# chorowski-lab/pytorch-asr

Hardware: AMD Instinct MI355X
Metric: CTC train-step frames/sec (higher is better)
Workload: dtype bf16; 1 GPU; WSJ mono-char CTC (egs/wsj/yamls/ctc.yaml shapes), DeepSpeech2 conv+4xBiLSTM-320 encoder + FSTDecoder, fwd+bwd+GradientClipping(clip 480000, skip 4.8e+06 = recipe x global_batch/16)+PolyakDecay+Adam, synthetic 40-dim x 1-channel x 1000-frame fbank; batch_per_gpu=768, global_batch=768, frames=1000, classes=49, parallelism=dp1, batch_norm=per-replica statistics, optimizer_steps=139, step_boundary=device: att_speech.fused_step (clip / skip decision + Adam, no read-back)

## Files before the change

### include/asr_amd.h

```cpp
#ifndef ASR_AMD_H
#define ASR_AMD_H

#include <stdint.h>

#ifdef __cplusplus
extern "C" {
#endif

enum {
    ASR_OK = 0,
    ASR_EINVAL = 1,
    ASR_EUNSUPPORTED = 2,
    ASR_ELAUNCH = 3
};

int asr_abi_version(void);

const char *asr_strerror(int code);

int64_t asr_lattice_fwbw_workspace_bytes(int T, int B, int C, int N);

int asr_lattice_fwbw_f32(const float *lp, int T, int B, int C,
                         const int32_t *lens,
                         const int32_t *src_in, const int32_t *il_in,
// ... 56 lines not shown
int asr_lattice_grouped_fwbw_f32(
    const float *lp, int T, int B, int C, const int32_t *lens, int N, int G, int Wg, int Wh,
    const int32_t *g_of, const int32_t *h_of, const int32_t *label, const int32_t *selfx,
    const int32_t *uniq, const int32_t *mem_g, const int32_t *mem_h, const float *term,
    float neg_inf, float *out_logZ, float *out_grad, float *out_logZ_bwd, void *workspace,
    int64_t workspace_bytes, void *stream);
int asr_lattice_grouped_fwbw_acc_f32(
    const float *lp, int T, int B, int C, const int32_t *lens, int N, int G, int Wg, int Wh,
    const int32_t *g_of, const int32_t *h_of, const int32_t *label, const int32_t *selfx,
    const int32_t *uniq, const int32_t *mem_g, const int32_t *mem_h, const float *term,
    float neg_inf, int accumulate, float *out_logZ, float *out_grad, float *out_logZ_bwd,
    void *workspace, int64_t workspace_bytes, void *stream);

int asr_lattice_grouped_forward_f32(
    const float *lp, int T, int B, int C, const int32_t *lens, int N, int G, int Wg, int Wh,
    const int32_t *g_of, const int32_t *h_of, const int32_t *label, const int32_t *selfx,
    const int32_t *uniq, const int32_t *mem_g, const int32_t *mem_h, const float *term,
    float neg_inf, int viterbi, float *out_score, int32_t *out_best_il, void *workspace,
    int64_t workspace_bytes, void *stream);

int64_t asr_lstm_workspace_bytes(int B, int H);

int asr_lstm_bidir_fwd_bf16(const void *gx, int gx_bf16, const void *whh_bf16,
                            const int32_t *lens, int T, int B, int H,
                            float *y, void *y_bf16, void *gates_bf16, float *csave,
                            void *workspace, int64_t workspace_bytes,
                            uint32_t *err_flag, void *stream);

int asr_lstm_wgrad_supported(int H);
int64_t asr_lstm_wgrad_workspace_bytes(int T, int B, int H, int with_input);
int asr_lstm_wgrad_bf16(const void *dgates_bf16, const void *x_bf16, const void *y_bf16,
                        int T, int B, int H, float *dw_ih, float *dw_hh,
                        void *workspace, int64_t workspace_bytes, void *stream);

int asr_lstm_dgrad_supported(int H);
int asr_lstm_dgrad_bf16(const void *dgates_bf16, const void *w_ih_bf16, int T, int B, int H,
                        float *dx, void *stream);

int asr_lstm_fused_supported(int B, int H, int F);
int asr_lstm_bidir_fwd_fused_bf16(const void *x_bf16, const void *wih_bf16,
                                  const void *whh_bf16, const int32_t *lens,
                                  int T, int B, int H, int F, float *y, void *y_bf16,
                                  void *gates_bf16, float *csave, void *workspace,
                                  int64_t workspace_bytes, uint32_t *err_flag, void *stream);

int asr_lstm_bidir_bwd_bf16(const float *dy, int dy_shared, const void *whhT_bf16,
                            const int32_t *lens, int T, int B, int H,
                            const void *gates_bf16, const float *csave,
                            void *dgates_bf16,
                            void *workspace, int64_t workspace_bytes,
                            uint32_t *err_flag, void *stream);

int64_t asr_gru_workspace_bytes(int B, int H);
int asr_gru_supported(int B, int H);

int asr_gru_bidir_fwd_bf16(const void *gx, int gx_bf16, const void *whh_bf16,
                           const int32_t *lens, int T, int B, int H,
                           float *y, void *y_bf16, void *gates_bf16,
                           void *workspace, int64_t workspace_bytes,
                           uint32_t *err_flag, void *stream);

int asr_gru_bidir_bwd_bf16(const float *dy, int dy_shared, const void *whhT_bf16,
                           const int32_t *lens, int T, int B, int H,
                           const void *gates_bf16, const float *y,
                           void *dgx_bf16, void *dhn_bf16,
                           void *workspace, int64_t workspace_bytes,
// ... 302 lines not shown
```

### pytorch-asr_amd/att_speech/_native.py

```python
import ctypes
import warnings
import os

import torch

_HERE = os.path.dirname(os.path.abspath(__file__))
LIB_PATH = os.environ.get(
    'ASR_AMD_LIB', os.path.join(os.path.dirname(_HERE), 'csrc', 'libasr_amd.so'))

ASR_OK, ASR_EINVAL, ASR_EUNSUPPORTED, ASR_ELAUNCH = 0, 1, 2, 3
ABI_VERSION = 24

_lib = None
EVENT_HOOK = None
_WARNED = {}

_vp, _i, _i64, _f = ctypes.c_void_p, ctypes.c_int, ctypes.c_int64, ctypes.c_float

_SIGNATURES = {
    'asr_abi_version': (ctypes.c_int, []),
    'asr_strerror': (ctypes.c_char_p, [_i]),
    'asr_lattice_fwbw_workspace_bytes': (_i64, [_i, _i, _i, _i]),
    'asr_lattice_fwbw_f32': (_i, [_vp, _i, _i, _i, _vp, _vp, _vp, _vp, _vp, _vp,
                                  _vp, _vp, _i, _i, _i, _i, _f, _vp, _vp, _vp,
# ... 75 lines not shown
    'asr_beam_lm_supported': (_i, [_i, _i, _i]),
    'asr_lm_label_costs_f64': (_i, [_vp, _vp, _vp, _i, _vp, _vp, _vp, _i, _vp, _vp, _i, _i, _i, _vp, _vp]),
    'asr_lm_bag_advance_f64': (_i, [_vp] * 6 + [_i, _i] + [_vp] * 7 + [_i, _vp, _vp, _vp, _i, _i, _i, _vp, _vp]),
    'asr_beam_lm_step_f32': (_i, [_vp, _vp, _vp, _vp, ctypes.c_double] + [_vp] * 7 + [_i] * 6 +
                             [_f, ctypes.c_double, _f, _f] + [_vp] * 15),
    'asr_graph_search_supported': (_i, [_i, _i, _i, _i]),
    'asr_beam_lm_step_graph_f32': (_i, [_vp, _vp, _vp, _vp, ctypes.c_double] + [_vp] * 7 + [_i] * 6 +
                                   [_f, ctypes.c_double, _f, _f] + [_vp] * 17),
    'asr_graph_merge_f32': (_i, [_vp] * 9 + [_i, _vp, _vp] + [_i] * 6 + [_f, _i] + [_vp] * 10),
    'asr_forced_level_f32': (_i, [_vp] * 11 + [_i] * 8 + [_f, _vp, _vp, _vp]),
    'asr_ctc_graph_build': (_i, [_vp, _vp, _i, _i, _i, _i, _i, _i, _f] + [_vp] * 8),
    'asr_lattice_grouped_workspace_bytes': (_i64, [_i, _i, _i, _i]),
    'asr_lattice_grouped_fwbw_f32': (_i, [_vp, _i, _i, _i, _vp, _i, _i, _i, _i] + [_vp] * 8 +
                                     [_f, _vp, _vp, _vp, _vp, _i64, _vp]),
    'asr_lattice_grouped_fwbw_acc_f32': (_i, [_vp, _i, _i, _i, _vp, _i, _i, _i, _i] + [_vp] * 8 +
                                         [_f, _i, _vp, _vp, _vp, _vp, _i64, _vp]),
    'asr_lattice_grouped_forward_f32': (_i, [_vp, _i, _i, _i, _vp, _i, _i, _i, _i] + [_vp] * 8 +
                                        [_f, _i, _vp, _vp, _vp, _i64, _vp]),
    'asr_lattice_shared_supported': (_i, [_i, _i, _i]),
    'asr_lattice_shared_workspace_bytes': (_i64, [_i, _i, _i]),
    'asr_lattice_shared_fwbw_f32': (_i, [_vp, _i, _i, _i, _vp, _i, _i] + [_vp] * 6 + [_i, _i, _vp, _i, _i,
                                         _f, _f, _i, _vp, _vp, _vp, _vp, _i64, _vp]),
    'asr_lattice_shared_forward_f32': (_i, [_vp, _i, _i, _i, _vp, _i, _i] + [_vp] * 4 +
                                       [_i, _i, _f, _i, _vp, _vp, _vp, _i64, _vp]),
    'asr_lstm_workspace_bytes': (_i64, [_i, _i]),
    'asr_lstm_bidir_fwd_bf16': (_i, [_vp, _i, _vp, _vp, _i, _i, _i, _vp, _vp, _vp, _vp, _vp, _i64, _vp, _vp]),
    'asr_lstm_bidir_bwd_bf16': (_i, [_vp, _i, _vp, _vp, _i, _i, _i, _vp, _vp, _vp, _vp, _i64, _vp, _vp]),
    'asr_lstm_fused_supported': (_i, [_i, _i, _i]),
    'asr_lstm_wgrad_supported': (_i, [_i]),
    'asr_lstm_dgrad_supported': (_i, [_i]),
    'asr_lstm_dgrad_bf16': (_i, [_vp, _vp, _i, _i, _i, _vp, _vp]),
    'asr_lstm_wgrad_workspace_bytes': (_i64, [_i, _i, _i, _i]),
    'asr_lstm_wgrad_bf16': (_i, [_vp, _vp, _vp, _i, _i, _i, _vp, _vp, _vp, _i64, _vp]),
    'asr_lstm_bidir_fwd_fused_bf16': (_i, [_vp, _vp, _vp, _vp, _i, _i, _i, _i, _vp, _vp, _vp, _vp, _vp, _i64, _vp, _vp]),
    'asr_gru_workspace_bytes': (_i64, [_i, _i]),
    'asr_gru_supported': (_i, [_i, _i]),
    'asr_gru_bidir_fwd_bf16': (_i, [_vp, _i, _vp, _vp, _i, _i, _i, _vp, _vp, _vp, _vp, _i64, _vp, _vp]),
    'asr_gru_bidir_bwd_bf16': (_i, [_vp, _i, _vp, _vp, _i, _i, _i, _vp, _vp, _vp, _vp, _vp, _i64, _vp, _vp]),
    'asr_bn_act_workspace_bytes': (_i64, [_i]),
    'asr_bn_act_fwd_f32': (_i, [_vp, _i, _vp, _i, _i, _i, _i, _vp, _vp, _vp, _vp, _i, _i, _f, _f, _f, _f,
                                _vp, _i, _i, _vp, _vp, _vp, _vp, _i64, _vp]),
    'asr_bn_act_bwd_f32': (_i, [_vp, _i, _vp, _i, _i, _i, _i, _vp, _vp, _vp, _vp, _i, _i, _f, _f,
                                _vp, _i, _i, _vp, _vp, _vp, _vp, _vp, _i64, _vp]),
    'asr_bn_act_bwd_phase_f32': (_i, [_vp, _i, _vp, _i, _i, _i, _i, _vp, _vp, _vp, _vp, _i, _i, _f, _f,
                                      _vp, _i, _i, _vp, _vp, _vp, _vp, _vp, _i64, _i, ctypes.c_double, _vp]),
}

_EXPERIMENT_SIGNATURES = {
    'asr_lstm_bidir_bwd_fused_bf16': (_i, [_vp, _i, _vp, _vp, _vp, _i, _i, _i, _vp, _vp, _vp, _vp,
                                           _vp, _i64, _vp, _vp]),
    'asr_lstm_bidir_fwd_fused_sum_bf16': (_i, [_vp, _vp, _vp, _vp, _i, _i, _i, _i, _vp, _vp, _vp, _vp, _vp, _vp, _i64,
                                               _vp, _vp]),
}
_experiments = False


class NativeLibraryError(RuntimeError):
    pass


def lib():
    global _lib, _experiments
    if _lib is None:
        if not os.path.exists(LIB_PATH):
            raise NativeLibraryError(
                "%s is missing: build it with `make -C pytorch-asr_amd/csrc` "
# ... 402 lines not shown
    if tuple(w_ih_bf16.shape) != (8 * H, H):
        raise ValueError('lstm_dgrad: w_ih must be [8H, H]')
    dx = torch.empty((T, B, H), dtype=torch.float32, device=dgates.device)
    check(lib().asr_lstm_dgrad_bf16(_p(dgates), _p(w_ih_bf16), T, B, H, _p(dx), _stream()),
          'asr_lstm_dgrad_bf16')
    return dx


def lstm_wgrad_supported(H):
    return bool(lib().asr_lstm_wgrad_supported(int(H)))


def lstm_wgrad(dgates, x_bf16, y_bf16):
    dgates = _dev(dgates, torch.bfloat16, 'dgates')
    y_bf16 = _dev(y_bf16, torch.bfloat16, 'y_bf16')
    T, B, H = dgates.shape[0], dgates.shape[1], dgates.shape[3] // 4
    dev = dgates.device
    if x_bf16 is not None:
        x_bf16 = _dev(x_bf16, torch.bfloat16, 'x')
        if x_bf16.numel() != T * B * H:
            raise ValueError('lstm_wgrad: x must be [T*B, H]')
    L = lib()
    dw_ih = torch.empty((8 * H, H), dtype=torch.float32, device=dev) if x_bf16 is not None else None
    dw_hh = torch.empty((2, 4 * H, H), dtype=torch.float32, device=dev)
    nbytes = L.asr_lstm_wgrad_workspace_bytes(T, B, H, int(x_bf16 is not None))
    if nbytes < 0:
        raise NativeLibraryError('asr_lstm_wgrad: unsupported hidden size %d' % H)
    ws = torch.empty(nbytes, dtype=torch.uint8, device=dev)
    check(L.asr_lstm_wgrad_bf16(_p(dgates), _p(x_bf16), _p(y_bf16), T, B, H, _p(dw_ih), _p(dw_hh),
                                _p(ws), nbytes, _stream()), 'asr_lstm_wgrad_bf16')
    return dw_ih, dw_hh


def _dy_mode(dy, planes):
    if planes:
        if dy.dim() != 4 or dy.shape[0] != 2:
            raise ValueError('dy planes must be [2,T,B,H]')
        return 2, dy.shape[1], dy.shape[2]
    return int(dy.dim() == 3), dy.shape[0], dy.shape[1]


def lstm_bidir_bwd(dy, whhT_bf16, lens, gates, csave, planes=False):
    dy = _dev(dy, torch.float32, 'dy')
    whhT_bf16 = _dev(whhT_bf16, torch.bfloat16, 'whhT')
    lens = _dev(lens, torch.int32, 'lens')
    mode, T, B = _dy_mode(dy, planes)
    H = dy.shape[-1]
    L = lib()
    dgates = torch.empty((T, B, 2, 4 * H), dtype=torch.bfloat16, device=dy.device)
    nbytes = L.asr_lstm_workspace_bytes(B, H)
    ws = torch.empty(nbytes, dtype=torch.uint8, device=dy.device)
    check(L.asr_lstm_bidir_bwd_bf16(_p(dy), mode, _p(whhT_bf16), _p(lens), T, B, H,
                                    _p(gates), _p(csave), _p(dgates), _p(ws), nbytes,
                                    _p(_lstm_err_flag(dy.device)), _stream()),
          'asr_lstm_bidir_bwd_bf16')
    return dgates


def lstm_bidir_bwd_fused(dy, whhT_bf16, wihT_bf16, lens, gates, csave, planes=False):
    dy = _dev(dy, torch.float32, 'dy')
    whhT_bf16 = _dev(whhT_bf16, torch.bfloat16, 'whhT')
    wihT_bf16 = _dev(wihT_bf16, torch.bfloat16, 'wihT')
    lens = _dev(lens, torch.int32, 'lens')
    _need_experiments('asr_lstm_bidir_bwd_fused_bf16')
    mode, T, B = _dy_mode(dy, planes)
    H = dy.shape[-1]
# ... 755 lines not shown
```

### pytorch-asr_amd/att_speech/modules/encoders/native_lstm.py

```python
import os

import torch

from att_speech import _native


def _mm_f32(a, b):
    try:
        return torch.mm(a, b, out_dtype=torch.float32)
    except (TypeError, RuntimeError):
        return torch.mm(a, b).float()


_FUSED_LIMITS = {'gates': 2 ** 32, 'planes': 2 ** 32, 'input': 2 ** 31}


def _fused_fits(T, B, H, F):
    return (T * B * 8 * H * 4 < _FUSED_LIMITS['gates'] and 2 * (T + 2) * B * H * 2 < _FUSED_LIMITS['planes']
            and T * B * F * 2 < _FUSED_LIMITS['input'])


def _forward_layer(xb, w_ih, whh, lens_dev, T, B, H, want_y, want_sum=False):
    F = xb.shape[1]
    mode = os.environ.get('ASR_LSTM_FUSED', '1')
# ... 36 lines not shown

class BiLSTMFunction(torch.autograd.Function):

    @staticmethod
    def forward(ctx, x, lens_dev, w_ih_f, w_hh_f, w_ih_r, w_hh_r, sum_dirs=False):
        T, B, F = x.shape
        H = w_hh_f.shape[1]
        xb = x.reshape(T * B, F).to(torch.bfloat16)
        ctx.x_bf16 = x.dtype == torch.bfloat16
        w_ih = torch.cat([w_ih_f, w_ih_r], 0).to(torch.bfloat16)
        whh = torch.stack([w_hh_f, w_hh_r], 0).to(torch.bfloat16).contiguous()
        y, ybf, gates, csave = _forward_layer(xb, w_ih, whh, lens_dev, T, B, H, True)
        ctx.save_for_backward(xb, lens_dev, w_ih, whh, ybf, gates, csave)
        return y.sum(2) if sum_dirs else y

    @staticmethod
    def backward(ctx, dy):
        xb, lens_dev, w_ih, whh, ybf, gates, csave = ctx.saved_tensors
        _, T2, B, H = ybf.shape
        T = T2 - 2
        F = xb.shape[1]
        whhT = whh.transpose(1, 2).contiguous()
        dgb = _native.lstm_bidir_bwd(dy.contiguous(), whhT, lens_dev, gates, csave)
        dx = _input_gradient(dgb, w_ih, T, B, H, F, bf16_out=ctx.x_bf16)
        dw_ih, dw_hh = _weight_gradients(dgb, xb, ybf, T, B, H, F)
        return dx, None, dw_ih[:4 * H], dw_hh[0], dw_ih[4 * H:], dw_hh[1], None


def _weight_gradients(dgb, xb, ybf, T, B, H, F):
    if os.environ.get('ASR_LSTM_WGRAD', '1') != '0' and _native.lstm_wgrad_supported(H) \
            and (T * B + 1024) * 16 * H < 2 ** 31:
        if F == H:
            dw_ih, dw_hh = _native.lstm_wgrad(dgb.view(T, B, 2, 4 * H), xb, ybf)
            return dw_ih, [dw_hh[0], dw_hh[1]]
        _, dw_hh = _native.lstm_wgrad(dgb.view(T, B, 2, 4 * H), None, ybf)
        TB = T * B
        g1 = _chunks(TB, 64)
        dw_ih = _native.sum_leading(_bmm_f32(dgb.view(g1, TB // g1, 8 * H).transpose(1, 2),
                                             xb.view(g1, TB // g1, F)))
        return dw_ih, [dw_hh[0], dw_hh[1]]
    return _weight_gradients_library(dgb, xb, ybf, T, B, H, F)


def _weight_gradients_library(dgb, xb, ybf, T, B, H, F):
    TB = T * B
    dg2 = dgb.view(TB, 8 * H)
    g1, g2 = _chunks(TB, 64), _chunks(TB, 32)
    dw_ih = _native.sum_leading(_bmm_f32(dg2.view(g1, TB // g1, 8 * H).transpose(1, 2),
                                         xb.view(g1, TB // g1, F)))
    dgd = dgb.view(g2, TB // g2, 2, 4 * H)
    dw_hh = [_native.sum_leading(_bmm_f32(
        dgd[:, :, d].transpose(1, 2),
        (ybf[0, 0:T] if d == 0 else ybf[1, 2:T + 2]).reshape(g2, TB // g2, H)))
        for d in range(2)]
    return dw_ih, dw_hh


class BiLSTMStackFunction(torch.autograd.Function):

    @staticmethod
    def forward(ctx, x, lens_dev, *weights):
        T, B, F = x.shape
        n = len(weights) // 4
        saved, xb = [], x.reshape(T * B, F).to(torch.bfloat16)
        ctx.x_bf16 = x.dtype == torch.bfloat16
        w_ihs, whhs, dst, src = [], [], [], []
# ... 66 lines not shown
```

### pytorch-asr_amd/csrc/lstm_wgrad.hip

```cpp
#include "common.h"
#include "../../include/asr_amd.h"

namespace {

typedef __attribute__((ext_vector_type(8))) __bf16 bf16x8;
typedef __attribute__((ext_vector_type(16))) float f32x16;
typedef __attribute__((ext_vector_type(4))) short s16x4;
typedef __attribute__((ext_vector_type(8))) short s16x8;
typedef __attribute__((ext_vector_type(4))) int rsrc_words;
typedef __attribute__((address_space(3))) s16x4 lds_s16x4;
typedef unsigned int u32;

constexpr int HN = 320;
constexpr int MT = 256;
constexpr int KT = 16;
constexpr int NS = 8;
constexpr int PA = MT * 2, PB = HN * 2;
constexpr int ACH = MT / 8, BCH = HN / 8;
constexpr int A_BYTES = KT * PA, B_BYTES = KT * PB;
constexpr int STAGE = A_BYTES + B_BYTES;
constexpr int A_DMA = KT * ACH / 64, B_DMA = KT * BCH / 64;
constexpr int PW = 3;
constexpr int DUMMY = NS * STAGE;
constexpr int LDS_BYTES = NS * STAGE + 1024;
constexpr int NMT = 8 * HN / MT;

struct WgradParams {
    const __bf16 *dg;
    const __bf16 *x;
    const __bf16 *hp[2];
    float *partial;
    int K;
    int rows_per_chunk;
    int njobs;
    int xcd_groups;
};

__device__ __forceinline__ void dma16(rsrc_words r, unsigned lds_byte, unsigned voff, unsigned soff) {
    unsigned keep;
    asm volatile("s_mov_b32 %0, m0\n\ts_mov_b32 m0, %1\n\ts_nop 0\n\t"
                 "buffer_load_dwordx4 %2, %3, %4 offen lds\n\ts_mov_b32 m0, %0"
                 : "=&s"(keep)
                 : "s"(lds_byte), "v"(voff), "s"(r), "s"(soff)
                 : "memory");
}
__device__ __forceinline__ unsigned lds_addr(const void *ptr) {
    return (unsigned)(size_t)((__attribute__((address_space(3))) const void *)ptr);
}
__device__ __forceinline__ bf16x8 tr_frag(const char *addr, int pitch4) {
    const s16x4 lo = __builtin_amdgcn_ds_read_tr16_b64_v4i16((lds_s16x4 *)(addr));
    const s16x4 hi = __builtin_amdgcn_ds_read_tr16_b64_v4i16((lds_s16x4 *)(addr + pitch4));
    s16x8 v;
    v.s0 = lo.x; v.s1 = lo.y; v.s2 = lo.z; v.s3 = lo.w;
    v.s4 = hi.x; v.s5 = hi.y; v.s6 = hi.z; v.s7 = hi.w;
    return __builtin_bit_cast(bf16x8, v);
}

__device__ __forceinline__ int swz_a(int chunk, int k) { return chunk ^ ((k & 3) << 2); }
__device__ __forceinline__ int swz_b(int chunk, int k) { return chunk ^ (((k & 3) >> 1) << 2); }

__global__ __launch_bounds__(512) void lstm_wgrad_kernel(WgradParams p) {
    extern __shared__ __attribute__((aligned(16))) char smem[];
    const int tid = threadIdx.x, lane = tid & 63;
    const int wave = __builtin_amdgcn_readfirstlane(tid >> 6);
    const int wm = wave >> 1, wn = wave & 1;
    int kc, job;
    if (p.xcd_groups) {
        const int w = blockIdx.x, per = p.njobs / 2;
        const int slot = w >> 3, grp = (w & 7) * p.xcd_groups + slot / per;
        kc = grp >> 1;
        job = (grp & 1) * per + slot % per;
    } else {
        job = blockIdx.x % p.njobs;
        kc = blockIdx.x / p.njobs;
    }
    const int per_dir = p.njobs / 2, dir = job / per_dir, jj = job % per_dir;
    const bool is_x = p.x != nullptr && jj < 5;
    const int mt = dir * 5 + (p.x != nullptr ? jj % 5 : jj);
    const __bf16 *bsrc = is_x ? p.x : p.hp[dir];
    const int k_begin = kc * p.rows_per_chunk, nstage = p.rows_per_chunk / KT;

    rsrc_words rs[PW];
    u32 voff[PW], lds_off[PW], soff[PW], stride[PW];
#pragma unroll
    for (int i = 0; i < PW; ++i) {
        const int q = wave + 8 * i;
        const bool isa = q < A_DMA, real = q < A_DMA + B_DMA;
        const unsigned long long base = (unsigned long long)(isa ? (const void *)p.dg : (const void *)bsrc);
        rs[i].x = __builtin_amdgcn_readfirstlane((int)(unsigned)base);
        rs[i].y = __builtin_amdgcn_readfirstlane((int)((unsigned)(base >> 32) & 0xffffu));
        rs[i].z = __builtin_amdgcn_readfirstlane(real ? (int)((u32)p.K * (isa ? 8 * HN * 2 : HN * 2)) : 0);
        rs[i].w = 0x00020000;
        stride[i] = isa ? KT * 8 * HN * 2 : KT * HN * 2;
        soff[i] = (u32)k_begin * (isa ? 8 * HN * 2 : HN * 2);
        lds_off[i] = real ? (u32)q * 1024u : (u32)DUMMY;
        if (isa) {
            const int L = 64 * q + lane, k = L / ACH, pos = L % ACH;
            voff[i] = (u32)k * (8 * HN * 2) + (u32)mt * PA + (u32)swz_a(pos, k) * 16u;
        } else {
            const int L = 64 * ((q - A_DMA) % B_DMA) + lane, k = L / BCH, pos = L % BCH;
            voff[i] = (u32)k * (HN * 2) + (u32)swz_b(pos, k) * 16u;
        }
    }
    u32 wslot = 0;
    const u32 smem_base = lds_addr(smem);
    auto issue_one = [&](int i) {
        dma16(rs[i], smem_base + wslot + lds_off[i], voff[i], soff[i]);
        soff[i] += stride[i];
    };
    auto issue_done = [&]() { wslot = wslot + STAGE == NS * STAGE ? 0u : wslot + STAGE; };

    const int g = lane >> 4, q4 = (lane & 15) >> 2, pp = lane & 3;
    const int krow = 8 * (g >> 1) + q4;
    u32 a_off[2], b_off[5];
#pragma unroll
    for (int i = 0; i < 2; ++i) {
        const int chunk = (wm * 64 + 32 * i) / 8 + 2 * (g & 1) + (pp >> 1);
        a_off[i] = (u32)krow * PA + (u32)swz_a(chunk, krow) * 16u + (u32)(pp & 1) * 8u;
    }
#pragma unroll
    for (int j = 0; j < 5; ++j) {
        const int chunk = (wn * 160 + 32 * j) / 8 + 2 * (g & 1) + (pp >> 1);
        b_off[j] = (u32)A_BYTES + (u32)krow * PB + (u32)swz_b(chunk, krow) * 16u + (u32)(pp & 1) * 8u;
    }
    f32x16 acc[2][5];
#pragma unroll
    for (int i = 0; i < 2; ++i)
#pragma unroll
        for (int j = 0; j < 5; ++j)
#pragma unroll
            for (int r = 0; r < 16; ++r) acc[i][j][r] = 0.f;
    bf16x8 fa[2][2], fb[2][5];
    u32 rslot = 0;

#define WG_MFMA(J) do { \
        acc[0][J] = __builtin_amdgcn_mfma_f32_32x32x16_bf16(a[0], b[J], acc[0][J], 0, 0, 0); \
        acc[1][J] = __builtin_amdgcn_mfma_f32_32x32x16_bf16(a[1], b[J], acc[1][J], 0, 0, 0); } while (0)
    auto step = [&](bf16x8 (&a)[2], bf16x8 (&b)[5], bf16x8 (&na)[2], bf16x8 (&nb)[5]) {
        asm volatile("s_waitcnt vmcnt(%0)\n\ts_barrier" ::"n"((NS - 3) * PW) : "memory");
        const char *rs_ = smem + rslot;
        WG_MFMA(0);
        na[0] = tr_frag(rs_ + a_off[0], 4 * PA);
        na[1] = tr_frag(rs_ + a_off[1], 4 * PA);
        __builtin_amdgcn_sched_barrier(0);
        WG_MFMA(1);
        nb[0] = tr_frag(rs_ + b_off[0], 4 * PB);
        nb[1] = tr_frag(rs_ + b_off[1], 4 * PB);
        issue_one(0);
        __builtin_amdgcn_sched_barrier(0);
        WG_MFMA(2);
        nb[2] = tr_frag(rs_ + b_off[2], 4 * PB);
        nb[3] = tr_frag(rs_ + b_off[3], 4 * PB);
        issue_one(1);
        __builtin_amdgcn_sched_barrier(0);
        WG_MFMA(3);
        nb[4] = tr_frag(rs_ + b_off[4], 4 * PB);
        issue_one(2);
        __builtin_amdgcn_sched_barrier(0);
        WG_MFMA(4);
        issue_done();
        rslot = rslot + STAGE == NS * STAGE ? 0u : rslot + STAGE;
        __builtin_amdgcn_sched_barrier(0);
    };
    for (int st = 0; st < NS - 1; ++st) {
#pragma unroll
        for (int i = 0; i < PW; ++i) issue_one(i);
        issue_done();
    }
    asm volatile("s_waitcnt vmcnt(%0)\n\ts_barrier" ::"n"((NS - 2) * PW) : "memory");
    fa[0][0] = tr_frag(smem + a_off[0], 4 * PA);
    fa[0][1] = tr_frag(smem + a_off[1], 4 * PA);
#pragma unroll
    for (int j = 0; j < 5; ++j) fb[0][j] = tr_frag(smem + b_off[j], 4 * PB);
    rslot = STAGE;
    for (int st = 0; st < nstage; st += 2) {
        step(fa[0], fb[0], fa[1], fb[1]);
        step(fa[1], fb[1], fa[0], fb[0]);
    }
#undef WG_MFMA
    asm volatile("s_waitcnt vmcnt(0)" ::: "memory");
    float *out = p.partial + ((((size_t)kc * p.njobs + job) * 8 + wave) * 10) * 1024;
#pragma unroll
    for (int i = 0; i < 2; ++i)
#pragma unroll
        for (int j = 0; j < 5; ++j)
#pragma unroll
            for (int r = 0; r < 16; ++r) out[((i * 5 + j) * 16 + r) * 64 + lane] = acc[i][j][r];
}

__global__ void lstm_wgrad_reduce_kernel(const float *partial, int nkc, int njobs, int with_x,
                                         float *dw_ih, float *dw_hh) {
    const size_t per = (size_t)njobs * 8 * 10 * 1024;
    const size_t idx = (size_t)blockIdx.x * blockDim.x + threadIdx.x;
    if (idx >= per) return;
    float s = 0.f;
    for (int kc = 0; kc < nkc; ++kc) s += partial[(size_t)kc * per + idx];
    const int lane = (int)(idx & 63), reg = (int)((idx >> 6) & 15);
    size_t rest = idx >> 10;
    const int tile = (int)(rest % 10); rest /= 10;
    const int wave = (int)(rest & 7), job = (int)(rest >> 3);
    const int per_dir = njobs / 2, dir = job / per_dir, jj = job % per_dir;
    const bool is_x = with_x && jj < 5;
    const int mt = dir * 5 + (with_x ? jj % 5 : jj);
    const int wm = wave >> 1, wn = wave & 1, i = tile / 5, j = tile % 5;
    const int row = (reg & 3) + 8 * (reg >> 2) + 4 * (lane >> 5);
    const int m = mt * MT + wm * 64 + 32 * i + row;
    const int n = wn * 160 + 32 * j + (lane & 31);
    (is_x ? dw_ih : dw_hh)[(size_t)m * HN + n] = s;
}

inline int cu_count() {
    int dev = 0, cus = 0;
    if (hipGetDevice(&dev) != hipSuccess) return 0;
    if (hipDeviceGetAttribute(&cus, hipDeviceAttributeMultiprocessorCount, dev) != hipSuccess) return 0;
    return cus;
}

struct Plan { int njobs, nkc, rows_per_chunk, xcd_groups; };
inline Plan make_plan(int K, int with_x) {
    Plan pl;
    pl.njobs = with_x ? 2 * NMT : NMT;
    int cus = cu_count();
    if (cus <= 0) cus = 256;
    pl.nkc = cus / pl.njobs > 0 ? cus / pl.njobs : 1;
    const int per_xcd = cus / 8, half = pl.njobs / 2;
    pl.xcd_groups = (cus % 8 == 0 && per_xcd >= half) ? per_xcd / half : 0;
    if (pl.xcd_groups) pl.nkc = 8 * pl.xcd_groups / 2;
    if (pl.nkc < 1) { pl.nkc = 1; pl.xcd_groups = 0; }
    const int per = (K + pl.nkc - 1) / pl.nkc;
    pl.rows_per_chunk = (per + 2 * KT - 1) / (2 * KT) * (2 * KT);
    if (pl.rows_per_chunk < 2 * KT) pl.rows_per_chunk = 2 * KT;
    return pl;
}

}

extern "C" int asr_lstm_wgrad_supported(int H) { return H == HN ? 1 : 0; }

extern "C" int64_t asr_lstm_wgrad_workspace_bytes(int T, int B, int H, int with_input) {
    if (T < 0 || B < 0 || H != HN) return -1;
    const Plan pl = make_plan(T * B, with_input);
    return (int64_t)pl.nkc * pl.njobs * 8 * 10 * 1024 * 4;
}

extern "C" int asr_lstm_wgrad_bf16(const void *dgates_bf16, const void *x_bf16, const void *y_bf16,
                                   int T, int B, int H, float *dw_ih, float *dw_hh,
                                   void *workspace, int64_t workspace_bytes, void *stream) {
    if (T <= 0 || B <= 0 || !dgates_bf16 || !y_bf16 || !dw_hh || !workspace) return ASR_EINVAL;
    if (H != HN) return ASR_EUNSUPPORTED;
    if ((x_bf16 == nullptr) != (dw_ih == nullptr)) return ASR_EINVAL;
    const int with_x = x_bf16 ? 1 : 0;
    const int64_t K = (int64_t)T * B;
    if ((K + 64 * KT) * 8 * HN * 2 >= (1ll << 31)) return ASR_EUNSUPPORTED;
    if (workspace_bytes < asr_lstm_wgrad_workspace_bytes(T, B, H, with_x)) return ASR_EINVAL;
    hipStream_t s = (hipStream_t)stream;
    const Plan pl = make_plan((int)K, with_x);
    WgradParams p;
    p.dg = (const __bf16 *)dgates_bf16;
    p.x = (const __bf16 *)x_bf16;
    const __bf16 *y = (const __bf16 *)y_bf16;
    p.hp[0] = y;
    p.hp[1] = y + ((size_t)(T + 2) + 2) * B * HN;
    p.partial = (float *)workspace;
    p.K = (int)K;
    p.rows_per_chunk = pl.rows_per_chunk;
    p.njobs = pl.njobs;
    p.xcd_groups = pl.xcd_groups;
    const size_t per = (size_t)pl.njobs * 8 * 10 * 1024;
    if (hipFuncSetAttribute((const void *)lstm_wgrad_kernel, hipFuncAttributeMaxDynamicSharedMemorySize,
                            LDS_BYTES) != hipSuccess)
        return ASR_ELAUNCH;
    hipLaunchKernelGGL(lstm_wgrad_kernel, dim3(pl.njobs * pl.nkc), dim3(512), LDS_BYTES, s, p);
    hipLaunchKernelGGL(lstm_wgrad_reduce_kernel, dim3((unsigned)((per + 255) / 256)), dim3(256), 0, s,
                       p.partial, pl.nkc, pl.njobs, with_x, dw_ih, dw_hh);
    return hipGetLastError() == hipSuccess ? ASR_OK : ASR_ELAUNCH;
}
```

Measured before the change: 36.62 million frames/s.

## Add native fused wgrad kernel for first LSTM layer with 352-wide input

Generalizes the LSTM weight-gradient MFMA kernel via a WIDE template so it also handles an input feature width of 352. Layer 0 can then compute dW_ih and dW_hh in one native launch instead of running the native dW_hh kernel plus a separate fallback GEMM for dW_ih. The path is on by default and can be turned off with ASR_LSTM_L0_NATIVE=0. In exchange it adds uneven work across wave columns (six tiles versus five), out-of-range DMA offsets for padding columns, and a larger workspace.

```diff
diff --git a/include/asr_amd.h b/include/asr_amd.h
--- a/include/asr_amd.h
+++ b/include/asr_amd.h
@@ -112,6 +112,12 @@
 int asr_lstm_wgrad_bf16(const void *dgates_bf16, const void *x_bf16, const void *y_bf16,
                         int T, int B, int H, float *dw_ih, float *dw_hh,
                         void *workspace, int64_t workspace_bytes, void *stream);
+
+int asr_lstm_wgrad_in_supported(int H, int F);
+int64_t asr_lstm_wgrad_in_workspace_bytes(int T, int B, int H, int F);
+int asr_lstm_wgrad_in_bf16(const void *dgates_bf16, const void *x_bf16, const void *y_bf16,
+                           int T, int B, int H, int F, float *dw_ih, float *dw_hh,
+                           void *workspace, int64_t workspace_bytes, void *stream);
 
 int asr_lstm_dgrad_supported(int H);
 int asr_lstm_dgrad_bf16(const void *dgates_bf16, const void *w_ih_bf16, int T, int B, int H,
diff --git a/pytorch-asr_amd/att_speech/_native.py b/pytorch-asr_amd/att_speech/_native.py
--- a/pytorch-asr_amd/att_speech/_native.py
+++ b/pytorch-asr_amd/att_speech/_native.py
@@ -131,6 +131,9 @@
     'asr_lstm_dgrad_bf16': (_i, [_vp, _vp, _i, _i, _i, _vp, _vp]),
     'asr_lstm_wgrad_workspace_bytes': (_i64, [_i, _i, _i, _i]),
     'asr_lstm_wgrad_bf16': (_i, [_vp, _vp, _vp, _i, _i, _i, _vp, _vp, _vp, _i64, _vp]),
+    'asr_lstm_wgrad_in_supported': (_i, [_i, _i]),
+    'asr_lstm_wgrad_in_workspace_bytes': (_i64, [_i, _i, _i, _i]),
+    'asr_lstm_wgrad_in_bf16': (_i, [_vp, _vp, _vp, _i, _i, _i, _i, _vp, _vp, _vp, _i64, _vp]),
     'asr_lstm_bidir_fwd_fused_bf16': (_i, [_vp, _vp, _vp, _vp, _i, _i, _i, _i, _vp, _vp, _vp, _vp, _vp, _i64, _vp, _vp]),
     'asr_gru_workspace_bytes': (_i64, [_i, _i]),
     'asr_gru_supported': (_i, [_i, _i]),
@@ -599,6 +602,31 @@
     return dw_ih, dw_hh
 
 
+def lstm_wgrad_in_supported(H, F):
+    return bool(lib().asr_lstm_wgrad_in_supported(int(H), int(F)))
+
+
+def lstm_wgrad_in(dgates, x_bf16, y_bf16):
+    dgates = _dev(dgates, torch.bfloat16, 'dgates')
+    y_bf16 = _dev(y_bf16, torch.bfloat16, 'y_bf16')
+    x_bf16 = _dev(x_bf16, torch.bfloat16, 'x')
+    T, B, H = dgates.shape[0], dgates.shape[1], dgates.shape[3] // 4
+    if x_bf16.dim() != 2 or x_bf16.shape[0] != T * B:
+        raise ValueError('lstm_wgrad_in: x must be [T*B, F]')
+    F = x_bf16.shape[1]
+    dev = dgates.device
+    L = lib()
+    nbytes = L.asr_lstm_wgrad_in_workspace_bytes(T, B, H, F)
+    if nbytes < 0:
+        raise NativeLibraryError('asr_lstm_wgrad_in: unsupported sizes H = %d, F = %d' % (H, F))
+    dw_ih = torch.empty((8 * H, F), dtype=torch.float32, device=dev)
+    dw_hh = torch.empty((2, 4 * H, H), dtype=torch.float32, device=dev)
+    ws = torch.empty(nbytes, dtype=torch.uint8, device=dev)
+    check(L.asr_lstm_wgrad_in_bf16(_p(dgates), _p(x_bf16), _p(y_bf16), T, B, H, F, _p(dw_ih), _p(dw_hh),
+                                   _p(ws), nbytes, _stream()), 'asr_lstm_wgrad_in_bf16')
+    return dw_ih, dw_hh
+
+
 def _dy_mode(dy, planes):
     if planes:
         if dy.dim() != 4 or dy.shape[0] != 2:
diff --git a/pytorch-asr_amd/att_speech/modules/encoders/native_lstm.py b/pytorch-asr_amd/att_speech/modules/encoders/native_lstm.py
--- a/pytorch-asr_amd/att_speech/modules/encoders/native_lstm.py
+++ b/pytorch-asr_amd/att_speech/modules/encoders/native_lstm.py
@@ -92,6 +92,9 @@
             and (T * B + 1024) * 16 * H < 2 ** 31:
         if F == H:
             dw_ih, dw_hh = _native.lstm_wgrad(dgb.view(T, B, 2, 4 * H), xb, ybf)
+            return dw_ih, [dw_hh[0], dw_hh[1]]
+        if os.environ.get('ASR_LSTM_L0_NATIVE', '1') != '0' and _native.lstm_wgrad_in_supported(H, F):
+            dw_ih, dw_hh = _native.lstm_wgrad_in(dgb.view(T, B, 2, 4 * H), xb, ybf)
             return dw_ih, [dw_hh[0], dw_hh[1]]
         _, dw_hh = _native.lstm_wgrad(dgb.view(T, B, 2, 4 * H), None, ybf)
         TB = T * B
diff --git a/pytorch-asr_amd/csrc/lstm_wgrad.hip b/pytorch-asr_amd/csrc/lstm_wgrad.hip
--- a/pytorch-asr_amd/csrc/lstm_wgrad.hip
+++ b/pytorch-asr_amd/csrc/lstm_wgrad.hip
@@ -12,18 +12,28 @@
 typedef unsigned int u32;
 
 constexpr int HN = 320;
+constexpr int FW = 352;
 constexpr int MT = 256;
 constexpr int KT = 16;
 constexpr int NS = 8;
-constexpr int PA = MT * 2, PB = HN * 2;
-constexpr int ACH = MT / 8, BCH = HN / 8;
-constexpr int A_BYTES = KT * PA, B_BYTES = KT * PB;
-constexpr int STAGE = A_BYTES + B_BYTES;
-constexpr int A_DMA = KT * ACH / 64, B_DMA = KT * BCH / 64;
+constexpr int PA = MT * 2;
+constexpr int ACH = MT / 8;
+constexpr int A_BYTES = KT * PA;
+constexpr int A_DMA = KT * ACH / 64;
 constexpr int PW = 3;
-constexpr int DUMMY = NS * STAGE;
-constexpr int LDS_BYTES = NS * STAGE + 1024;
 constexpr int NMT = 8 * HN / MT;
+template <bool WIDE> struct Geo {
+    static constexpr int NB = WIDE ? FW : HN;
+    static constexpr int PB = NB * 2;
+    static constexpr int BCH = NB / 8;
+    static constexpr int B_BYTES = KT * PB;
+    static constexpr int STAGE = A_BYTES + B_BYTES;
+    static constexpr int B_DMA = KT * BCH / 64;
+    static constexpr int DUMMY = NS * STAGE;
+    static constexpr int LDS_BYTES = NS * STAGE + 1024;
+    static constexpr int NT = WIDE ? 6 : 5;
+    static_assert(A_DMA + B_DMA <= 8 * PW && LDS_BYTES <= 160 * 1024, "stage does not fit");
+};
 
 struct WgradParams {
     const __bf16 *dg;
@@ -59,11 +69,18 @@
 __device__ __forceinline__ int swz_a(int chunk, int k) { return chunk ^ ((k & 3) << 2); }
 __device__ __forceinline__ int swz_b(int chunk, int k) { return chunk ^ (((k & 3) >> 1) << 2); }
 
+template <bool WIDE> __device__ __host__ __forceinline__ int wave_col(int wave) {
+    return WIDE ? (wave ^ (wave >> 2)) & 1 : wave & 1;
+}
+
+template <bool WIDE>
 __global__ __launch_bounds__(512) void lstm_wgrad_kernel(WgradParams p) {
+    using G = Geo<WIDE>;
+    constexpr int PB = G::PB, BCH = G::BCH, STAGE = G::STAGE, B_DMA = G::B_DMA, DUMMY = G::DUMMY;
     extern __shared__ __attribute__((aligned(16))) char smem[];
     const int tid = threadIdx.x, lane = tid & 63;
     const int wave = __builtin_amdgcn_readfirstlane(tid >> 6);
-    const int wm = wave >> 1, wn = wave & 1;
+    const int wm = wave >> 1, wn = wave_col<WIDE>(wave);
     int kc, job;
     if (p.xcd_groups) {
         const int w = blockIdx.x, per = p.njobs / 2;
@@ -79,6 +96,7 @@
     const int mt = dir * 5 + (p.x != nullptr ? jj % 5 : jj);
     const __bf16 *bsrc = is_x ? p.x : p.hp[dir];
     const int k_begin = kc * p.rows_per_chunk, nstage = p.rows_per_chunk / KT;
+    const int bcols = WIDE && is_x ? FW : HN, bpitch = bcols * 2;
 
     rsrc_words rs[PW];
     u32 voff[PW], lds_off[PW], soff[PW], stride[PW];
@@ -89,124 +107,208 @@
         const unsigned long long base = (unsigned long long)(isa ? (const void *)p.dg : (const void *)bsrc);
         rs[i].x = __builtin_amdgcn_readfirstlane((int)(unsigned)base);
         rs[i].y = __builtin_amdgcn_readfirstlane((int)((unsigned)(base >> 32) & 0xffffu));
-        rs[i].z = __builtin_amdgcn_readfirstlane(real ? (int)((u32)p.K * (isa ? 8 * HN * 2 : HN * 2)) : 0);
+        rs[i].z = __builtin_amdgcn_readfirstlane(real ? (int)((u32)p.K * (isa ? 8 * HN * 2 : bpitch)) : 0);
         rs[i].w = 0x00020000;
-        stride[i] = isa ? KT * 8 * HN * 2 : KT * HN * 2;
-        soff[i] = (u32)k_begin * (isa ? 8 * HN * 2 : HN * 2);
+        stride[i] = isa ? KT * 8 * HN * 2 : KT * bpitch;
+        soff[i] = (u32)k_begin * (isa ? 8 * HN * 2 : bpitch);
         lds_off[i] = real ? (u32)q * 1024u : (u32)DUMMY;
         if (isa) {
             const int L = 64 * q + lane, k = L / ACH, pos = L % ACH;
             voff[i] = (u32)k * (8 * HN * 2) + (u32)mt * PA + (u32)swz_a(pos, k) * 16u;
+        } else if (!WIDE) {
+            const int L = 64 * ((q - A_DMA) % B_DMA) + lane, k = L / BCH, pos = L % BCH;
+            voff[i] = (u32)k * (HN * 2) + (u32)swz_b(pos, k) * 16u;
         } else {
             const int L = 64 * ((q - A_DMA) % B_DMA) + lane, k = L / BCH, pos = L % BCH;
-            voff[i] = (u32)k * (HN * 2) + (u32)swz_b(pos, k) * 16u;
+            voff[i] = pos * 8 < bcols ? (u32)k * bpitch + (u32)pos * 16u : 0x7ff00000u;
         }
     }
     u32 wslot = 0;
     const u32 smem_base = lds_addr(smem);
     auto issue_one = [&](int i) {
-        dma16(rs[i], smem_base + wslot + lds_off[i], voff[i], soff[i]);
+        if constexpr (WIDE)
+            dma16(rs[i], smem_base + (lds_off[i] == (u32)DUMMY ? 0u : wslot) + lds_off[i], voff[i], soff[i]);
+        else
+            dma16(rs[i], smem_base + wslot + lds_off[i], voff[i], soff[i]);
         soff[i] += stride[i];
     };
     auto issue_done = [&]() { wslot = wslot + STAGE == NS * STAGE ? 0u : wslot + STAGE; };
 
     const int g = lane >> 4, q4 = (lane & 15) >> 2, pp = lane & 3;
     const int krow = 8 * (g >> 1) + q4;
-    u32 a_off[2], b_off[5];
+    u32 a_off[2];
 #pragma unroll
     for (int i = 0; i < 2; ++i) {
         const int chunk = (wm * 64 + 32 * i) / 8 + 2 * (g & 1) + (pp >> 1);
         a_off[i] = (u32)krow * PA + (u32)swz_a(chunk, krow) * 16u + (u32)(pp & 1) * 8u;
     }
-#pragma unroll
-    for (int j = 0; j < 5; ++j) {
-        const int chunk = (wn * 160 + 32 * j) / 8 + 2 * (g & 1) + (pp >> 1);
-        b_off[j] = (u32)A_BYTES + (u32)krow * PB + (u32)swz_b(chunk, krow) * 16u + (u32)(pp & 1) * 8u;
-    }
-    f32x16 acc[2][5];
-#pragma unroll
-    for (int i = 0; i < 2; ++i)
-#pragma unroll
-        for (int j = 0; j < 5; ++j)
-#pragma unroll
-            for (int r = 0; r < 16; ++r) acc[i][j][r] = 0.f;
-    bf16x8 fa[2][2], fb[2][5];
-    u32 rslot = 0;
-
 #define WG_MFMA(J) do { \
         acc[0][J] = __builtin_amdgcn_mfma_f32_32x32x16_bf16(a[0], b[J], acc[0][J], 0, 0, 0); \
         acc[1][J] = __builtin_amdgcn_mfma_f32_32x32x16_bf16(a[1], b[J], acc[1][J], 0, 0, 0); } while (0)
-    auto step = [&](bf16x8 (&a)[2], bf16x8 (&b)[5], bf16x8 (&na)[2], bf16x8 (&nb)[5]) {
-        asm volatile("s_waitcnt vmcnt(%0)\n\ts_barrier" ::"n"((NS - 3) * PW) : "memory");
-        const char *rs_ = smem + rslot;
-        WG_MFMA(0);
-        na[0] = tr_frag(rs_ + a_off[0], 4 * PA);
-        na[1] = tr_frag(rs_ + a_off[1], 4 * PA);
-        __builtin_amdgcn_sched_barrier(0);
-        WG_MFMA(1);
-        nb[0] = tr_frag(rs_ + b_off[0], 4 * PB);
-        nb[1] = tr_frag(rs_ + b_off[1], 4 * PB);
-        issue_one(0);
-        __builtin_amdgcn_sched_barrier(0);
-        WG_MFMA(2);
-        nb[2] = tr_frag(rs_ + b_off[2], 4 * PB);
-        nb[3] = tr_frag(rs_ + b_off[3], 4 * PB);
-        issue_one(1);
-        __builtin_amdgcn_sched_barrier(0);
-        WG_MFMA(3);
-        nb[4] = tr_frag(rs_ + b_off[4], 4 * PB);
-        issue_one(2);
-        __builtin_amdgcn_sched_barrier(0);
-        WG_MFMA(4);
-        issue_done();
-        rslot = rslot + STAGE == NS * STAGE ? 0u : rslot + STAGE;
-        __builtin_amdgcn_sched_barrier(0);
-    };
-    for (int st = 0; st < NS - 1; ++st) {
-#pragma unroll
-        for (int i = 0; i < PW; ++i) issue_one(i);
-        issue_done();
-    }
-    asm volatile("s_waitcnt vmcnt(%0)\n\ts_barrier" ::"n"((NS - 2) * PW) : "memory");
-    fa[0][0] = tr_frag(smem + a_off[0], 4 * PA);
-    fa[0][1] = tr_frag(smem + a_off[1], 4 * PA);
-#pragma unroll
-    for (int j = 0; j < 5; ++j) fb[0][j] = tr_frag(smem + b_off[j], 4 * PB);
-    rslot = STAGE;
-    for (int st = 0; st < nstage; st += 2) {
-        step(fa[0], fb[0], fa[1], fb[1]);
-        step(fa[1], fb[1], fa[0], fb[0]);
+    if constexpr (!WIDE) {
+        u32 b_off[5];
+#pragma unroll
+        for (int j = 0; j < 5; ++j) {
+            const int chunk = (wn * 160 + 32 * j) / 8 + 2 * (g & 1) + (pp >> 1);
+            b_off[j] = (u32)A_BYTES + (u32)krow * PB + (u32)swz_b(chunk, krow) * 16u + (u32)(pp & 1) * 8u;
+        }
+        f32x16 acc[2][5];
+#pragma unroll
+        for (int i = 0; i < 2; ++i)
+#pragma unroll
+            for (int j = 0; j < 5; ++j)
+#pragma unroll
+                for (int r = 0; r < 16; ++r) acc[i][j][r] = 0.f;
+        bf16x8 fa[2][2], fb[2][5];
+        u32 rslot = 0;
+
+        auto step = [&](bf16x8 (&a)[2], bf16x8 (&b)[5], bf16x8 (&na)[2], bf16x8 (&nb)[5]) {
+            asm volatile("s_waitcnt vmcnt(%0)\n\ts_barrier" ::"n"((NS - 3) * PW) : "memory");
+            const char *rs_ = smem + rslot;
+            WG_MFMA(0);
+            na[0] = tr_frag(rs_ + a_off[0], 4 * PA);
+            na[1] = tr_frag(rs_ + a_off[1], 4 * PA);
+            __builtin_amdgcn_sched_barrier(0);
+            WG_MFMA(1);
+            nb[0] = tr_frag(rs_ + b_off[0], 4 * PB);
+            nb[1] = tr_frag(rs_ + b_off[1], 4 * PB);
+            issue_one(0);
+            __builtin_amdgcn_sched_barrier(0);
+            WG_MFMA(2);
+            nb[2] = tr_frag(rs_ + b_off[2], 4 * PB);
+            nb[3] = tr_frag(rs_ + b_off[3], 4 * PB);
+            issue_one(1);
+            __builtin_amdgcn_sched_barrier(0);
+            WG_MFMA(3);
+            nb[4] = tr_frag(rs_ + b_off[4], 4 * PB);
+            issue_one(2);
+            __builtin_amdgcn_sched_barrier(0);
+            WG_MFMA(4);
+            issue_done();
+            rslot = rslot + STAGE == NS * STAGE ? 0u : rslot + STAGE;
+            __builtin_amdgcn_sched_barrier(0);
+        };
+        for (int st = 0; st < NS - 1; ++st) {
+#pragma unroll
+            for (int i = 0; i < PW; ++i) issue_one(i);
+            issue_done();
+        }
+        asm volatile("s_waitcnt vmcnt(%0)\n\ts_barrier" ::"n"((NS - 2) * PW) : "memory");
+        fa[0][0] = tr_frag(smem + a_off[0], 4 * PA);
+        fa[0][1] = tr_frag(smem + a_off[1], 4 * PA);
+#pragma unroll
+        for (int j = 0; j < 5; ++j) fb[0][j] = tr_frag(smem + b_off[j], 4 * PB);
+        rslot = STAGE;
+        for (int st = 0; st < nstage; st += 2) {
+            step(fa[0], fb[0], fa[1], fb[1]);
+            step(fa[1], fb[1], fa[0], fb[0]);
+        }
+        asm volatile("s_waitcnt vmcnt(0)" ::: "memory");
+        float *out = p.partial + ((((size_t)kc * p.njobs + job) * 8 + wave) * 10) * 1024;
+#pragma unroll
+        for (int i = 0; i < 2; ++i)
+#pragma unroll
+            for (int j = 0; j < 5; ++j)
+#pragma unroll
+                for (int r = 0; r < 16; ++r) out[((i * 5 + j) * 16 + r) * 64 + lane] = acc[i][j][r];
+    } else {
+        const int col0 = wn * (is_x ? 192 : 160);
+        const bool six = is_x && wn == 0;
+        const u32 b_off = (u32)A_BYTES + (u32)krow * PB + (u32)(col0 / 8 + 2 * (g & 1) + (pp >> 1)) * 16u +
+                          (u32)(pp & 1) * 8u;
+        f32x16 acc[2][6];
+#pragma unroll
+        for (int i = 0; i < 2; ++i)
+#pragma unroll
+            for (int j = 0; j < 6; ++j)
+#pragma unroll
+                for (int r = 0; r < 16; ++r) acc[i][j][r] = 0.f;
+        bf16x8 fa[2][2], b[6];
+        u32 rslot = 0;
+        auto step = [&](bf16x8 (&a)[2], bf16x8 (&na)[2]) {
+            asm volatile("s_waitcnt vmcnt(%0)\n\ts_barrier" ::"n"((NS - 3) * PW) : "memory");
+            const char *rs_ = smem + rslot;
+            WG_MFMA(0);
+            na[0] = tr_frag(rs_ + a_off[0], 4 * PA);
+            na[1] = tr_frag(rs_ + a_off[1], 4 * PA);
+            __builtin_amdgcn_sched_barrier(0);
+            WG_MFMA(1);
+            b[0] = tr_frag(rs_ + b_off, 4 * PB);
+            b[1] = tr_frag(rs_ + b_off + 64, 4 * PB);
+            issue_one(0);
+            __builtin_amdgcn_sched_barrier(0);
+            WG_MFMA(2);
+            b[2] = tr_frag(rs_ + b_off + 128, 4 * PB);
+            issue_one(1);
+            __builtin_amdgcn_sched_barrier(0);
+            WG_MFMA(3);
+            b[3] = tr_frag(rs_ + b_off + 192, 4 * PB);
+            issue_one(2);
+            __builtin_amdgcn_sched_barrier(0);
+            WG_MFMA(4);
+            b[4] = tr_frag(rs_ + b_off + 256, 4 * PB);
+            __builtin_amdgcn_sched_barrier(0);
+            if (six) {
+                WG_MFMA(5);
+                b[5] = tr_frag(rs_ + b_off + 320, 4 * PB);
+                __builtin_amdgcn_sched_barrier(0);
+            }
+            issue_done();
+            rslot = rslot + STAGE == NS * STAGE ? 0u : rslot + STAGE;
+            __builtin_amdgcn_sched_barrier(0);
+        };
+        for (int st = 0; st < NS - 1; ++st) {
+#pragma unroll
+            for (int i = 0; i < PW; ++i) issue_one(i);
+            issue_done();
+        }
+        asm volatile("s_waitcnt vmcnt(%0)\n\ts_barrier" ::"n"((NS - 2) * PW) : "memory");
+        fa[0][0] = tr_frag(smem + a_off[0], 4 * PA);
+        fa[0][1] = tr_frag(smem + a_off[1], 4 * PA);
+#pragma unroll
+        for (int j = 0; j < 5; ++j) b[j] = tr_frag(smem + b_off + 64 * j, 4 * PB);
+        b[5] = six ? tr_frag(smem + b_off + 320, 4 * PB) : b[4];
+        rslot = STAGE;
+        for (int st = 0; st < nstage; st += 2) {
+            step(fa[0], fa[1]);
+            step(fa[1], fa[0]);
+        }
+        asm volatile("s_waitcnt vmcnt(0)" ::: "memory");
+        float *out = p.partial + ((((size_t)kc * p.njobs + job) * 8 + wave) * 12) * 1024;
+#pragma unroll
+        for (int i = 0; i < 2; ++i)
+#pragma unroll
+            for (int j = 0; j < 6; ++j)
+                if (j < 5 || six) {
+#pragma unroll
+                    for (int r = 0; r < 16; ++r) out[((i * 6 + j) * 16 + r) * 64 + lane] = acc[i][j][r];
+                }
     }
 #undef WG_MFMA
-    asm volatile("s_waitcnt vmcnt(0)" ::: "memory");
-    float *out = p.partial + ((((size_t)kc * p.njobs + job) * 8 + wave) * 10) * 1024;
-#pragma unroll
-    for (int i = 0; i < 2; ++i)
-#pragma unroll
-        for (int j = 0; j < 5; ++j)
-#pragma unroll
-            for (int r = 0; r < 16; ++r) out[((i * 5 + j) * 16 + r) * 64 + lane] = acc[i][j][r];
-}
-
+}
+
+template <bool WIDE>
 __global__ void lstm_wgrad_reduce_kernel(const float *partial, int nkc, int njobs, int with_x,
                                          float *dw_ih, float *dw_hh) {
-    const size_t per = (size_t)njobs * 8 * 10 * 1024;
+    constexpr int NT = Geo<WIDE>::NT;
+    const size_t per = (size_t)njobs * 8 * (2 * NT) * 1024;
     const size_t idx = (size_t)blockIdx.x * blockDim.x + threadIdx.x;
     if (idx >= per) return;
-    float s = 0.f;
-    for (int kc = 0; kc < nkc; ++kc) s += partial[(size_t)kc * per + idx];
     const int lane = (int)(idx & 63), reg = (int)((idx >> 6) & 15);
     size_t rest = idx >> 10;
-    const int tile = (int)(rest % 10); rest /= 10;
+    const int tile = (int)(rest % (2 * NT)); rest /= 2 * NT;
     const int wave = (int)(rest & 7), job = (int)(rest >> 3);
     const int per_dir = njobs / 2, dir = job / per_dir, jj = job % per_dir;
     const bool is_x = with_x && jj < 5;
     const int mt = dir * 5 + (with_x ? jj % 5 : jj);
-    const int wm = wave >> 1, wn = wave & 1, i = tile / 5, j = tile % 5;
+    const int wm = wave >> 1, wn = wave_col<WIDE>(wave), i = tile / NT, j = tile % NT;
+    if (WIDE && j == 5 && !(is_x && wn == 0)) return;
+    float s = 0.f;
+    for (int kc = 0; kc < nkc; ++kc) s += partial[(size_t)kc * per + idx];
     const int row = (reg & 3) + 8 * (reg >> 2) + 4 * (lane >> 5);
     const int m = mt * MT + wm * 64 + 32 * i + row;
-    const int n = wn * 160 + 32 * j + (lane & 31);
-    (is_x ? dw_ih : dw_hh)[(size_t)m * HN + n] = s;
+    const int n = wn * (WIDE && is_x ? 192 : 160) + 32 * j + (lane & 31);
+    (is_x ? dw_ih : dw_hh)[(size_t)m * (WIDE && is_x ? FW : HN) + n] = s;
 }
 
 inline int cu_count() {
@@ -233,27 +335,12 @@
     return pl;
 }
 
-}
-
-extern "C" int asr_lstm_wgrad_supported(int H) { return H == HN ? 1 : 0; }
-
-extern "C" int64_t asr_lstm_wgrad_workspace_bytes(int T, int B, int H, int with_input) {
-    if (T < 0 || B < 0 || H != HN) return -1;
-    const Plan pl = make_plan(T * B, with_input);
-    return (int64_t)pl.nkc * pl.njobs * 8 * 10 * 1024 * 4;
-}
-
-extern "C" int asr_lstm_wgrad_bf16(const void *dgates_bf16, const void *x_bf16, const void *y_bf16,
-                                   int T, int B, int H, float *dw_ih, float *dw_hh,
-                                   void *workspace, int64_t workspace_bytes, void *stream) {
-    if (T <= 0 || B <= 0 || !dgates_bf16 || !y_bf16 || !dw_hh || !workspace) return ASR_EINVAL;
-    if (H != HN) return ASR_EUNSUPPORTED;
-    if ((x_bf16 == nullptr) != (dw_ih == nullptr)) return ASR_EINVAL;
+template <bool WIDE>
+int wgrad_launch(const void *dgates_bf16, const void *x_bf16, const void *y_bf16, int T, int B,
+                 float *dw_ih, float *dw_hh, void *workspace, hipStream_t s) {
+    using G = Geo<WIDE>;
     const int with_x = x_bf16 ? 1 : 0;
     const int64_t K = (int64_t)T * B;
-    if ((K + 64 * KT) * 8 * HN * 2 >= (1ll << 31)) return ASR_EUNSUPPORTED;
-    if (workspace_bytes < asr_lstm_wgrad_workspace_bytes(T, B, H, with_x)) return ASR_EINVAL;
-    hipStream_t s = (hipStream_t)stream;
     const Plan pl = make_plan((int)K, with_x);
     WgradParams p;
     p.dg = (const __bf16 *)dgates_bf16;
@@ -266,12 +353,60 @@
     p.rows_per_chunk = pl.rows_per_chunk;
     p.njobs = pl.njobs;
     p.xcd_groups = pl.xcd_groups;
-    const size_t per = (size_t)pl.njobs * 8 * 10 * 1024;
-    if (hipFuncSetAttribute((const void *)lstm_wgrad_kernel, hipFuncAttributeMaxDynamicSharedMemorySize,
-                            LDS_BYTES) != hipSuccess)
+    const size_t per = (size_t)pl.njobs * 8 * (2 * G::NT) * 1024;
+    if (hipFuncSetAttribute((const void *)lstm_wgrad_kernel<WIDE>, hipFuncAttributeMaxDynamicSharedMemorySize,
+                            G::LDS_BYTES) != hipSuccess)
         return ASR_ELAUNCH;
-    hipLaunchKernelGGL(lstm_wgrad_kernel, dim3(pl.njobs * pl.nkc), dim3(512), LDS_BYTES, s, p);
-    hipLaunchKernelGGL(lstm_wgrad_reduce_kernel, dim3((unsigned)((per + 255) / 256)), dim3(256), 0, s,
+    hipLaunchKernelGGL(lstm_wgrad_kernel<WIDE>, dim3(pl.njobs * pl.nkc), dim3(512), G::LDS_BYTES, s, p);
+    hipLaunchKernelGGL(lstm_wgrad_reduce_kernel<WIDE>, dim3((unsigned)((per + 255) / 256)), dim3(256), 0, s,
                        p.partial, pl.nkc, pl.njobs, with_x, dw_ih, dw_hh);
     return hipGetLastError() == hipSuccess ? ASR_OK : ASR_ELAUNCH;
 }
+
+inline bool offsets_fit(int64_t K) { return (K + 64 * KT) * 8 * HN * 2 < (1ll << 31); }
+
+}
+
+extern "C" int asr_lstm_wgrad_supported(int H) { return H == HN ? 1 : 0; }
+
+extern "C" int64_t asr_lstm_wgrad_workspace_bytes(int T, int B, int H, int with_input) {
+    if (T < 0 || B < 0 || H != HN) return -1;
+    const Plan pl = make_plan(T * B, with_input);
+    return (int64_t)pl.nkc * pl.njobs * 8 * 10 * 1024 * 4;
+}
+
+extern "C" int asr_lstm_wgrad_bf16(const void *dgates_bf16, const void *x_bf16, const void *y_bf16,
+                                   int T, int B, int H, float *dw_ih, float *dw_hh,
+                                   void *workspace, int64_t workspace_bytes, void *stream) {
+    if (T <= 0 || B <= 0 || !dgates_bf16 || !y_bf16 || !dw_hh || !workspace) return ASR_EINVAL;
+    if (H != HN) return ASR_EUNSUPPORTED;
+    if ((x_bf16 == nullptr) != (dw_ih == nullptr)) return ASR_EINVAL;
+    if (!offsets_fit((int64_t)T * B)) return ASR_EUNSUPPORTED;
+    if (workspace_bytes < asr_lstm_wgrad_workspace_bytes(T, B, H, x_bf16 ? 1 : 0)) return ASR_EINVAL;
+    return wgrad_launch<false>(dgates_bf16, x_bf16, y_bf16, T, B, dw_ih, dw_hh, workspace,
+                               (hipStream_t)stream);
+}
+
+extern "C" int asr_lstm_wgrad_in_supported(int H, int F) { return H == HN && (F == HN || F == FW) ? 1 : 0; }
+
+extern "C" int64_t asr_lstm_wgrad_in_workspace_bytes(int T, int B, int H, int F) {
+    if (T < 0 || B < 0 || !asr_lstm_wgrad_in_supported(H, F)) return -1;
+    if (F == HN) return asr_lstm_wgrad_workspace_bytes(T, B, H, 1);
+    const Plan pl = make_plan(T * B, 1);
+    return (int64_t)pl.nkc * pl.njobs * 8 * (2 * Geo<true>::NT) * 1024 * 4;
+}
+
+extern "C" int asr_lstm_wgrad_in_bf16(const void *dgates_bf16, const void *x_bf16, const void *y_bf16,
+                                      int T, int B, int H, int F, float *dw_ih, float *dw_hh,
+                                      void *workspace, int64_t workspace_bytes, void *stream) {
+    if (T <= 0 || B <= 0 || !dgates_bf16 || !x_bf16 || !y_bf16 || !dw_ih || !dw_hh || !workspace)
+        return ASR_EINVAL;
+    if (!asr_lstm_wgrad_in_supported(H, F)) return ASR_EUNSUPPORTED;
+    if (!offsets_fit((int64_t)T * B)) return ASR_EUNSUPPORTED;
+    if (workspace_bytes < asr_lstm_wgrad_in_workspace_bytes(T, B, H, F)) return ASR_EINVAL;
+    if (F == HN)
+        return wgrad_launch<false>(dgates_bf16, x_bf16, y_bf16, T, B, dw_ih, dw_hh, workspace,
+                                   (hipStream_t)stream);
+    return wgrad_launch<true>(dgates_bf16, x_bf16, y_bf16, T, B, dw_ih, dw_hh, workspace,
+                              (hipStream_t)stream);
+}
```

Result: no change. 37.17 million frames/s, median of 6 (+1.5%).
